# zhangzhousuper/Radish_PT

Measured on AMD Instinct MI355X. Metric: Mrays/s, higher is better.
Workload: dtype f32

## Files before the change

### radish_pt_amd/csrc/device/kernels_wave.h

```cpp
#pragma once
#include "kernels_pt.h"
#include "wg_trace.h"
#include "ray_cull.h"

namespace rd {

constexpr int kWfLitCap = 8192;
constexpr int kWfLitShadow = 0x40000000;
constexpr int kMaxWaveDepth = 32;

struct alignas(128) WaveCounter {
    int v;
    int pad[31];
};
#ifndef RD_WF_TICKET_SHARDS
#define RD_WF_TICKET_SHARDS 8
#endif
constexpr int kTicketShards = RD_WF_TICKET_SHARDS;
struct WaveCounters {
    WaveCounter rayCount[kMaxWaveDepth + 2];
    WaveCounter shadowCount[kMaxWaveDepth + 2];
    WaveCounter litCount[kMaxWaveDepth + 2];
    WaveCounter litShadowCount[kMaxWaveDepth + 2];
    WaveCounter traceHead[kMaxWaveDepth + 2];
    WaveCounter shadeHead[kMaxWaveDepth + 2][4];
    WaveCounter traceTicket[kMaxWaveDepth + 2][kTicketShards];
    WaveCounter shadeTicket[kMaxWaveDepth + 2][kTicketShards];
};

struct WaveWorkspace {
    float4 *ro[2];
    float4 *rd[2];
    float4 *thr[2];
    float4 *prevPos[2];
    float4 *accD;
    float4 *accI;
    float4 *nee[2];
    float4 *sht[2];
    uint2 *rng[2];
    int4 *hit;
    int *rayq[2];
    int *shadowq;
    int *litq[2];
    int litCap;
    int *treeOvf;
    int treeOvfDepth;
#ifdef RD_WF_STAMPS
    unsigned long long *stamps;
    int stampWaves;
    int stampStages;
#endif
    WaveCounters *ctr;
};

constexpr unsigned kWfNeeNone = 2u;
RD_DEV float wfNeeTag(int home, unsigned kind) { return __uint_as_float(((unsigned)home << 2) | kind); }
RD_DEV void wfAddNee(const WaveWorkspace &w, float4 n) {
    const unsigned tag = __float_as_uint(n.w), kind = tag & 3u;
    if (kind == kWfNeeNone) return;
    float4 *acc = (kind == 0u ? w.accD : w.accI) + (tag >> 2);
    const float4 a = *acc;
    *acc = make_float4(a.x + n.x, a.y + n.y, a.z + n.z, 0.f);
}

RD_DEV Ray wfSlotRay(const WaveWorkspace &w, int set, int p, bool shadow, float &limit) {
    if (shadow) {
        const float4 x = w.prevPos[set][p], y = w.sht[set][p];
        return shadowRay(mk3(x.x, x.y, x.z), mk3(y.x, y.y, y.z), limit);
    }
    const float4 o = w.ro[set][p], d = w.rd[set][p];
    limit = 3.402823466e+38f;
    return Ray{mk3(o.x, o.y, o.z), mk3(d.x, d.y, d.z)};
}

struct WaveSlotPath {
    const WaveWorkspace &w;
    const int rs, p;
    const int wr, q;
    int home;
    const bool delta;
    bool nullNee = false;
    RD_DEV v3 throughput() {
        const float4 t = w.thr[rs][p];
        home = __float_as_int(t.w);
        return mk3(t.x, t.y, t.z);
    }
    RD_DEV float samplePdf() const { return w.ro[rs][p].w; }
    RD_DEV bool sampleDelta() const { return delta; }
    RD_DEV v3 prevPos() const { const float4 c = w.prevPos[rs][p]; return mk3(c.x, c.y, c.z); }
    RD_DEV void setDirect(v3 v) { w.accD[home] = make_float4(v.x, v.y, v.z, 0.f); }
    RD_DEV void addIndirect(v3 v) { const float4 a = w.accI[home]; w.accI[home] = make_float4(a.x + v.x, a.y + v.y, a.z + v.z, 0.f); }
    RD_DEV Sampler rng(const DScene &s) const { const uint2 r = w.rng[rs][p]; return Sampler{s.sobol, r.x, (int)r.y}; }
    RD_DEV void setNee(v3 c, float nw) {
        w.nee[wr][q] = make_float4(c.x, c.y, c.z, wfNeeTag(home, nw < 0.f ? kWfNeeNone : (nw == 0.f ? 0u : 1u)));
        nullNee = nw < 0.f || (c.x == 0.f && c.y == 0.f && c.z == 0.f);
    }
    RD_DEV void setPrevPos(v3 x) { w.prevPos[wr][q] = make_float4(x.x, x.y, x.z, 0.f); }
    RD_DEV void setRay(const Ray &ray, float pdf, bool deltaSample, v3 throughput, const Sampler &rng) {
        w.ro[wr][q] = make_float4(ray.o.x, ray.o.y, ray.o.z, pdf);
        w.rd[wr][q] = make_float4(ray.d.x, ray.d.y, ray.d.z, deltaSample ? 1.f : 0.f);
        w.thr[wr][q] = make_float4(throughput.x, throughput.y, throughput.z, __int_as_float(home));
        w.rng[wr][q] = make_uint2(rng.scramble, (unsigned)rng.ptr);
    }
};


RD_DEV void waveAppend(bool pred, int item, int *queue, int *count) {
    unsigned long long mask = __ballot(pred);
    if (mask == 0ull) return;
    int leader = __ffsll((long long)mask) - 1;
    int base = 0;
    if ((int)(threadIdx.x & 63u) == leader) base = atomicAdd(count, __popcll(mask));
    base = __shfl(base, leader, 64);
    if (pred) queue[base + __popcll(mask & laneMaskLt())] = item;
}

constexpr int kShadeChunks = 4;
constexpr int kShadePacket = 64 * kShadeChunks;
RD_DEV void waveAppendN(const bool (&pred)[kShadeChunks], const int (&item)[kShadeChunks], int *queue, int *count) {
    unsigned long long m[kShadeChunks];
    int total = 0;
#pragma unroll
    for (int j = 0; j < kShadeChunks; j++) {
        m[j] = __ballot(pred[j]);
        total += __popcll(m[j]);
    }
    if (total == 0) return;
    int base = 0;
    if ((threadIdx.x & 63u) == 0u) base = atomicAdd(count, total);
    base = __shfl(base, 0, 64);
#pragma unroll
    for (int j = 0; j < kShadeChunks; j++) {
        if (pred[j]) queue[base + __popcll(m[j] & laneMaskLt())] = item[j];
        base += __popcll(m[j]);
    }
}

constexpr int kPacket = 128;
RD_DEV int gridWaves() { return int(gridDim.x * (blockDim.x >> 6)); }
RD_DEV int workgroupTicket(WaveCounter *tickets) {
    __shared__ int ticket;
    if (threadIdx.x == 0) {
        const unsigned x = blockIdx.x % (unsigned)kTicketShards;
        ticket = int(x + (unsigned)kTicketShards * (unsigned)atomicAdd(&tickets[x].v, 1));
    }
    __syncthreads();
    return __builtin_amdgcn_readfirstlane(ticket);
}
RD_DEV int logicalWave(int wg) { return __builtin_amdgcn_readfirstlane(int(wg * int(blockDim.x >> 6) + int(threadIdx.x >> 6))); }
RD_DEV int wavePull(int *head, int packet) {
    int base = 0;
    if ((threadIdx.x & 63u) == 0u) base = atomicAdd(head, packet);
    return __shfl(base, 0, 64) + gridWaves() * packet;
}
RD_DEV int tracePull(int *head, int headBase) {
    int base = 0;
    if ((threadIdx.x & 63u) == 0u) base = atomicAdd(head, kPacket);
    return __builtin_amdgcn_readlane(base, 0) + headBase;
}

RD_DEV unsigned subFrameBlocks(const PixelMap &pm, int part, int parts) { return (unsigned)(pm.numBlocks - part + parts - 1) / (unsigned)parts; }
constexpr int kSobolRows = 10000;
__global__ __launch_bounds__(256) void k_wf_raygen(DScene s, DCamera cam, PixelMap pm, WaveWorkspace w, int looper, int samples, int part,
                                                   int parts) {
    unsigned wg;
    const unsigned nLocal = subFrameBlocks(pm, part, parts);
    const unsigned nGroups = nLocal * (unsigned)samples;
    bool wgValid = xcdSwizzle(blockIdx.x, (nGroups + 3u) >> 2, wg);
    unsigned lane = threadIdx.x & 63u;
    unsigned group = wgValid ? wg * 4u + (threadIdx.x >> 6) : 0xffffffffu / 64u;
    const bool inRange = wgValid && group < nGroups;
    const unsigned b = group / nLocal, blockLocal = group - b * nLocal;
    Pix px = mapPixel(pm, inRange ? blockLocal * (unsigned)parts + (unsigned)part : 0xffffffffu / 64u, lane);
    bool valid = px.valid && inRange;
    int p = int(group * 64u + lane);
    bool listed = false;
    if (valid) {
        Sampler rng = makeSeededRandomEngine(int(((unsigned)looper + b) % (unsigned)kSobolRows), px.index, 0, s.sobol);
        Ray ray = cameraSample(cam, px.x, px.y, sample4D(rng));
        w.ro[0][p] = make_float4(ray.o.x, ray.o.y, ray.o.z, 0.f);
        w.rd[0][p] = make_float4(ray.d.x, ray.d.y, ray.d.z, 0.f);
        w.accD[p] = make_float4(0.f, 0.f, 0.f, 0.f);
        w.accI[p] = make_float4(0.f, 0.f, 0.f, 0.f);
        w.rng[0][p] = make_uint2(rng.scramble, (unsigned)rng.ptr);
        if (fabs_(ray.d.x) < 1.1e-6f || fabs_(ray.d.y) < 1.1e-6f || fabs_(ray.d.z) < 1.1e-6f) {
            const int at = atomicAdd(&w.ctr->litCount[0].v, 1);
            if (at < w.litCap) {
                w.litq[0][at] = p;
                listed = true;
            }
        }
    }
    if (inRange) w.rayq[0][p] = valid ? (listed ? -2 - p : p) : -1;
    if (blockIdx.x == 0 && threadIdx.x == 0) w.ctr->rayCount[0].v = int(nGroups) * 64;
}

#ifndef RD_WF_DUTY_SHARE
#define RD_WF_DUTY_SHARE 0
#endif
#ifndef RD_REFILL_MIN
#define RD_REFILL_MIN 16
#endif
#ifndef RD_WF_FINISH_MIN
#define RD_WF_FINISH_MIN 16
#endif
#ifndef RD_WF_SHADOW_FIRST
#define RD_WF_SHADOW_FIRST 0
#endif
constexpr int kWfStampKinds = 6;
#ifdef RD_WF_STAMPS
#define RD_WF_STAMP(kind) do { if (stampAt && (threadIdx.x & 63u) == 0u) stampAt[kind] = wall_clock64(); } while (0)
#define RD_WF_STAMP_DRY() do { if (exhausted && !stampedDry) { stampedDry = true; RD_WF_STAMP(1); if (stampAt && (threadIdx.x & 63u) == 0u) *headDry = 1ull; } } while (0)
#define RD_WF_STAMP_HELD(held) do { if (stampAt && !stampedHeld && *headDry != 0ull) { \
        stampedHeld = true; const int h_ = (held); if ((threadIdx.x & 63u) == 0u) stampAt[4] = 1ull + (unsigned long long)h_; } } while (0)
#else
#define RD_WF_STAMP(kind) ((void)0)
#define RD_WF_STAMP_DRY() ((void)0)
#define RD_WF_STAMP_HELD(held) ((void)0)
#endif
#ifndef RD_WF_COOP_LONE
#define RD_WF_COOP_LONE 1
#endif

#ifndef RD_WF_TRACE_WAVES
#define RD_WF_TRACE_WAVES 7
#endif
#ifndef RD_WF_PAIR_WAVES
#define RD_WF_PAIR_WAVES 1
#endif
#ifndef RD_WF_PAIR_MAX_WAVES
#define RD_WF_PAIR_MAX_WAVES 6
#endif
template <bool COUNT, bool PAIRS = false>
__global__ __launch_bounds__(256) __attribute__((amdgpu_waves_per_eu(PAIRS && !COUNT ? RD_WF_PAIR_WAVES : (!COUNT ? RD_WF_TRACE_WAVES : 1),
                                                                      PAIRS && !COUNT ? RD_WF_PAIR_MAX_WAVES : 8))) void k_wf_trace(DScene s, WaveWorkspace w, int k) {
    WaveCounters *c = w.ctr;
    const int wg = workgroupTicket(c->traceTicket[k]);
#ifdef RD_WF_STAMPS
    unsigned long long *const stampAt = w.stamps ? w.stamps + ((size_t)k * (size_t)w.stampWaves + (size_t)logicalWave(wg)) * kWfStampKinds : nullptr;
    volatile unsigned long long *const headDry = w.stamps ? w.stamps + (size_t)w.stampStages * (size_t)w.stampWaves * kWfStampKinds + k : nullptr;
    bool stampedDry = false, stampedHeld = false;
    RD_WF_STAMP(0);
#endif
    const int nShadow = (k > 0) ? c->shadowCount[k - 1].v : 0;
    const int nRay = c->rayCount[k].v;
    const int total = nShadow + nRay;
    const int *rayq = w.rayq[k & 1];
    const int set = k & 1;
    WalkStats ws{0, 0};
    unsigned nClosest = 0, nAny = 0, nHits = 0;
    const int end = s.bvhSize;
    const int END = end;

    const int nLit = c->litCount[k].v < w.litCap ? c->litCount[k].v : w.litCap;
    const int dutyGroups = RD_WF_DUTY_SHARE ? 0 : (nLit < int(gridDim.x) ? nLit : int(gridDim.x));
    const bool duty = wg < dutyGroups;
    const int headBase = (int(gridDim.x) - dutyGroups) * int(blockDim.x >> 6) * kPacket;
    int resNext = duty ? headBase : (logicalWave(wg) - dutyGroups * int(blockDim.x >> 6)) * kPacket, resEnd = duty ? resNext : resNext + kPacket;
    bool exhausted = resNext >= total;
    if (resEnd > total) resEnd = total;
    RD_WF_STAMP_DRY();

    bool alive = false;
    bool isShadow = false;
    int p = -1;
    RaySlab rs;
    rs.o = rs.d = rs.inv = mk3(0.f);
    rs.cls = 0;
    const NodeRec *nodes = s.nodes[0];
    int ord = 0, cur = kPairNone;
    PairStack sp{0, 0};
    int node = END, pending = -1;
    float tmax = 0.f;
    int hitPrim = -1;
    v2 hitBary = mk2(0.f, 0.f);
    bool occluded = false;

    constexpr int kStackEntries = PAIRS ? 4 * kPairLds * 64 : 1;
    __shared__ union WfTraceLds {
        WgTraceSharedT<256> wg;
        int2 stack[kStackEntries];
    } lds;
    WgTraceSharedT<256> &wgsh = lds.wg;
    int2 *const stk = lds.stack + (PAIRS ? int(threadIdx.x >> 6) * kPairLds * 64 : 0);
    int2 *const ovf = PAIRS ? reinterpret_cast<int2 *>(w.treeOvf) + (size_t)logicalWave(wg) * (size_t)w.treeOvfDepth * 64 : nullptr;
    for (int it = wg; it < nLit; it += int(gridDim.x)) {
        const int e = w.litq[k & 1][it];
        const bool sh = (e & kWfLitShadow) != 0;
        const int pp = e & (kWfLitShadow - 1);
        float lim;
        const Ray ray = wfSlotRay(w, set, pp, sh, lim);
        const RaySlab urs = makeRaySlab(ray);
        if (urs.cls == 0 || end == 0) continue;
        const NodeRec *un = s.nodes[getMTBVHId(-ray.d)];
        const CoopTrace ct = sh ? wgTraceWhole<true, 256>(s, un, urs, lim, wgsh) : wgTraceWhole<false, 256>(s, un, urs, lim, wgsh);
        if (threadIdx.x == 0) {
            if (sh) {
                nAny++;
                if (!ct.found) wfAddNee(w, w.nee[set][pp]);
            } else {
                nClosest++;
                const bool hit = ct.hitPrim != -1;
                if (hit) nHits++;
                w.hit[pp] = make_int4(ct.hitPrim, __float_as_int(hit ? ct.bary.x : 0.f), __float_as_int(hit ? ct.bary.y : 0.f),
                                      hit ? int(s.primClass[ct.hitPrim]) : 0);
            }
            if (COUNT) {
                ws.nodes += ct.nodes;
                ws.tris += ct.tris;
            }
        }
    }
    RD_WF_STAMP(3);
#ifdef RD_WF_STAMPS
    if (stampAt && (threadIdx.x & 63u) == 0u) stampAt[5] = 1ull + (unsigned long long)nLit;
#endif
    if (PAIRS) __syncthreads();
    bool firstRound = true;
    bool fromList = false;
    for (;;) {
        bool doStart = false;
        fromList = false;
        if (firstRound) {
            firstRound = false;
            const int it = wg + (int(threadIdx.x & 63u) * 4 + int(threadIdx.x >> 6)) * int(gridDim.x);
            if (it < nLit) {
                const int e = w.litq[k & 1][it];
                doStart = true;
                fromList = true;
                isShadow = (e & kWfLitShadow) != 0;
                p = e & (kWfLitShadow - 1);
            }
        }
        unsigned long long idle = __ballot(!alive && !doStart && p < 0);
        int nIdle = __popcll(idle);
        if (!exhausted && nIdle >= RD_REFILL_MIN) {
            RD_WF_STAMP_HELD(resEnd - resNext);
            int myRank = __popcll(idle & laneMaskLt());
            int taken = 0;
            while (taken < nIdle && !exhausted) {
                if (resNext == resEnd) {
                    resNext = tracePull(&c->traceHead[k].v, headBase);
                    resEnd = resNext + kPacket;
                    if (resNext >= total) {
                        exhausted = true;
                        break;
                    }
                    if (resEnd > total) resEnd = total;
                }
                int avail = resEnd - resNext;
                int give = (nIdle - taken) < avail ? (nIdle - taken) : avail;
                if (!alive && !doStart && p < 0 && myRank >= taken && myRank < taken + give) {
                    const int item = resNext + (myRank - taken);
                    doStart = true;
#if RD_WF_SHADOW_FIRST
                    isShadow = item < nShadow;
                    p = isShadow ? w.shadowq[item] : rayq[item - nShadow];
#else
                    isShadow = item >= nRay;
                    p = isShadow ? w.shadowq[item - nRay] : rayq[item];
#endif
                }
                resNext += give;
                taken += give;
            }
        }
        RD_WF_STAMP_DRY();
        if (doStart) {
            if (p >= 0) {
                const Ray ray = wfSlotRay(w, set, p, isShadow, tmax);
                if (isShadow) nAny++;
                else nClosest++;
                rs = makeRaySlab(ray);
                pending = -1;
                if (PAIRS) {
                    ord = getMTBVHId(-ray.d);
                    sp = PairStack{0, 0};
                    if (rs.cls == 0 || end == 0) pairStart<COUNT>(s, rs, tmax, cur, pending, ws);
                    else cur = kPairFresh;
                    alive = true;
                } else {
                    nodes = s.nodes[getMTBVHId(-ray.d)];
                    node = 0;
                    alive = node != END;
                }
                hitPrim = -1;
                occluded = false;
                if (fromList && rs.cls != 0 && end != 0) {
                    if (isShadow) nAny--;
                    else nClosest--;
                    alive = false;
                    p = -1;
                }
            }
        }
        unsigned long long am = __ballot(alive);
        if (am == 0ull) {
            if (exhausted) break;
            continue;
        }

        {
            unsigned long long lit = __ballot(PAIRS ? (alive && cur == kPairFresh) : (alive && rs.cls != 0 && node == 0 && pending < 0));
            while (lit) {
                const int L = __ffsll((long long)lit) - 1;
                lit &= lit - 1ull;
                const bool shadowL = readlaneI(isShadow ? 1 : 0, L) != 0;
                const NodeRec *un = PAIRS ? s.nodes[0] + (size_t)readlaneI(ord, L) * (size_t)(end + 1) : readlanePtr(nodes, L);
                const RaySlab ur = readlaneRay(rs, L);
                const float lim = readlaneF(tmax, L);
                CoopTrace ct = shadowL ? coopTraceWhole<true>(s, un, ur, lim) : coopTraceWhole<false>(s, un, ur, lim);
                if (int(threadIdx.x & 63u) == L) {
                    hitPrim = ct.hitPrim;
                    hitBary = ct.bary;
                    tmax = ct.tmax;
                    occluded = ct.found;
                    node = END;
                    cur = kPairNone;
                    alive = false;
                    if (COUNT) {
                        ws.nodes += ct.nodes;
                        ws.tris += ct.tris;
                    }
                }
            }
        }
        if (PAIRS) {
            bool busy = alive && pending < 0;
            const int nStart = __popcll(__ballot(busy));
            if (nStart > 0) {
                const int minWalk = (nStart * (RD_LEAF_DEN - RD_LEAF_NUM) + RD_LEAF_DEN - 1) / RD_LEAF_DEN;
                const int lane = int(threadIdx.x & 63u);
                do {
                    pairPopOne<COUNT>(stk, lane, ovf, tmax, busy, cur, sp, pending, ws);
                    if (busy && cur >= 0) {
                        pairStep<COUNT>(s.pairs, stk, lane, ovf, rs, tmax, ord, cur, sp, pending, ws);
                        busy = pending < 0 && (cur >= 0 || sp.sp > 0);
                    }
                } while (__popcll(__ballot(busy)) >= (minWalk > 1 ? minWalk : 1));
                alive = alive && (pending >= 0 || cur >= 0 || sp.sp > 0);
            }
        } else
        {
            bool walking = alive && pending < 0;
            const int nStart = __popcll(__ballot(walking));
#if RD_WF_COOP_LONE
            if (nStart == 1) {
                const int L = __ffsll((long long)__ballot(walking)) - 1;
                CoopResult cr = coopWalk(readlanePtr(nodes, L), readlaneI(node, L), end, readlaneRay(rs, L), readlaneF(tmax, L), RD_COOP_WINDOWS);
                if (int(threadIdx.x & 63u) == L) {
                    node = cr.node;
                    pending = cr.pending;
                    if (COUNT) ws.nodes += cr.visited;
                    alive = (node != end) || pending >= 0;
                }
            } else
#endif
            if (nStart > 0) {
                const int minWalk = (nStart * (RD_LEAF_DEN - RD_LEAF_NUM) + RD_LEAF_DEN - 1) / RD_LEAF_DEN;
                do {
                    if (walking) {
                        if (COUNT) ws.nodes++;
                        float4 lo = nodes[node].lo_prim;
                        float4 hi = nodes[node].hi_next;
                        float boundDist;
                        bool boundHit = aabbFast(lo, hi, rs, boundDist);
                        if (boundHit && boundDist < tmax) {
                            pending = __float_as_int(lo.w);
                            node++;
                        } else {
                            node = __float_as_int(hi.w);
                        }
                        walking = pending < 0 && node != END;
                        alive = (node != END) || pending >= 0;
                    }
                } while (__popcll(__ballot(walking)) >= (minWalk > 1 ? minWalk : 1));
            }
        }
        if (alive && pending >= 0) {
            TriVerts t = loadTri(s.tris, pending);
            float dist;
            v2 bary;
            if (COUNT) ws.tris++;
            bool hit = intersectTriangle(rs, t.a, t.b, t.c, bary, dist);
            if (hit && dist < tmax) {
                if (isShadow) {
                    occluded = true;
                    node = END;
                    cur = kPairNone;
                    sp = PairStack{0, 0};
                } else {
                    hitPrim = pending;
                    tmax = dist;
                    hitBary = bary;
                }
            }
            pending = -1;
            alive = PAIRS ? (cur >= 0 || sp.sp > 0) : (node != END);
        }
        const unsigned long long doneM = __ballot(!alive && p >= 0);
        if (doneM != 0ull && __popcll(doneM) * 64 >= (__popcll(doneM) + __popcll(__ballot(alive))) * RD_WF_FINISH_MIN)
        if (!alive && p >= 0) {
            if (isShadow) {
                if (!occluded) wfAddNee(w, w.nee[set][p]);
            } else {
                bool hit = hitPrim != -1;
                if (hit) nHits++;
                w.hit[p] = make_int4(hitPrim, __float_as_int(hit ? hitBary.x : 0.f), __float_as_int(hit ? hitBary.y : 0.f),
                                     hit ? int(s.primClass[hitPrim]) : 0);
            }
            p = -1;
        }
    }
    RD_WF_STAMP(2);
    if (COUNT) flushCounters(s.counters, nClosest, nAny, nHits, ws);
}

constexpr int kSortChunks = 16;
constexpr int kSortPacket = 64 * kSortChunks;
#ifndef RD_WF_SHADE_WAVES
#define RD_WF_SHADE_WAVES 1
#endif
#ifndef RD_WF_CULL_LAST
#define RD_WF_CULL_LAST 1
#endif
#ifndef RD_WF_SKIP_NULL_NEE
#define RD_WF_SKIP_NULL_NEE 1
#endif
__global__ __launch_bounds__(256, RD_WF_SHADE_WAVES) void k_wf_shade(DScene s, WaveWorkspace w, int k, int maxDepth, int sorted,
                                                                     const float4 *__restrict__ emitBox, int walkAll) {
    __shared__ int sSorted[4][kSortPacket];
    WaveCounters *c = w.ctr;
    const bool cullLast = RD_WF_CULL_LAST && !walkAll && k + 1 == maxDepth && !hasEnvMap(s);
    const bool skipNull = RD_WF_SKIP_NULL_NEE && !walkAll;
    float4 boxLo = make_float4(0.f, 0.f, 0.f, 0.f), boxHi = boxLo;
    if (cullLast) {
        boxLo = emitBox[0];
        boxHi = emitBox[1];
    }
    const int wg = workgroupTicket(c->shadeTicket[k]);
    const int lane = int(threadIdx.x & 63u);
    int *mySorted = sSorted[threadIdx.x >> 6];
    {
        const int q = 0;
        const int n = c->rayCount[k].v;
        const int *hitq = w.rayq[k & 1];
        int pendP[kShadeChunks], pendQ[kShadeChunks];
        bool pendShadow[kShadeChunks], pendRay[kShadeChunks];
#pragma unroll
        for (int j = 0; j < kShadeChunks; j++) {
            pendP[j] = pendQ[j] = -1;
            pendShadow[j] = pendRay[j] = false;
        }
        int packet = kShadePacket;
        if (sorted) {
            const int perWave = n / (2 * gridWaves());
            packet = ((perWave + kShadePacket - 1) / kShadePacket) * kShadePacket;
            packet = packet < kShadePacket ? kShadePacket : (packet > kSortPacket ? kSortPacket : packet);
        }
        int packetEnd = 0;
        for (int base = logicalWave(wg) * packet, sub = 0, fresh = 1;;) {
            if (sub == packet) {
                base = wavePull(&c->shadeHead[k][q].v, packet);
                sub = 0;
                fresh = 1;
            }
            if (base + sub >= n) break;
            if (sorted && fresh) {
                fresh = 0;
                packetEnd = (n - base) < packet ? (n - base) : packet;
                int pp[kSortChunks], cls[kSortChunks];
#pragma unroll
                for (int j = 0; j < kSortChunks; j++) {
                    const int i = base + j * 64 + lane;
                    pp[j] = (j * 64 + lane < packetEnd) ? hitq[i] : -1;
                    if (pp[j] <= -2) pp[j] = -2 - pp[j];
                }
#pragma unroll
                for (int j = 0; j < kSortChunks; j++) {
                    cls[j] = (pp[j] >= 0) ? w.hit[pp[j]].w : 0;
                }
                int at = 0;
#pragma unroll
                for (int qq = 0; qq < 4; qq++) {
#pragma unroll
                    for (int j = 0; j < kSortChunks; j++) {
                        const bool in = (j * 64 + lane < packetEnd) && cls[j] == qq;
                        const unsigned long long m = __ballot(in);
                        if (in) mySorted[at + __popcll(m & laneMaskLt())] = pp[j];
                        at += __popcll(m);
                    }
                }
                __builtin_amdgcn_wave_barrier();
            }
            int item = base + sub + lane;
            const int subNow = sub;
            sub += 64;
            bool active = sorted ? (subNow + lane < packetEnd) : (item < n);
            bool emitShadow = false, emitRay = false, litShadow = false, litRay = false, rayFirst = false;
            int p = -1;
            const int q = base + subNow + lane;
            if (active) {
                p = sorted ? mySorted[subNow + lane] : hitq[item];
                if (p <= -2) p = -2 - p;
                active = p >= 0;
            }
            if (active) {
                const int4 h = w.hit[p];
                const float4 rdw = w.rd[k & 1][p];
                WaveSlotPath st{w, k & 1, p, (k + 1) & 1, q, p, rdw.w != 0.f};
                const PathStepResult r = pathStep(s, k, maxDepth, h.x, mk2(__int_as_float(h.y), __int_as_float(h.z)), mk3(rdw.x, rdw.y, rdw.z), st);
                if (r.shadow && !(skipNull && st.nullNee)) {
                    w.sht[(k + 1) & 1][q] = make_float4(r.shadowTo.x, r.shadowTo.y, r.shadowTo.z, 0.f);
                    emitShadow = true;
                    const v3 dl = r.shadowTo - r.shadowFrom;
                    const float l2 = dot(dl, dl) * 1.21e-12f;
                    litShadow = dl.x * dl.x < l2 || dl.y * dl.y < l2 || dl.z * dl.z < l2;
                }
                if (r.extension && !(cullLast && !mayReachEmitters(boxLo, boxHi, r.ray.o, r.ray.d))) {
                    emitRay = true;
                    litRay = fabs_(r.ray.d.x) < 1.1e-6f || fabs_(r.ray.d.y) < 1.1e-6f || fabs_(r.ray.d.z) < 1.1e-6f;
                }
            }
            if (__ballot(litShadow || litRay) != 0ull) {
                int *lq = w.litq[(k + 1) & 1];
                int *lc = &c->litCount[k + 1].v;
                for (int kind = 0; kind < 2; kind++) {
                    const bool pred = kind == 0 ? litShadow : litRay;
                    const unsigned long long m = __ballot(pred);
                    if (m == 0ull) continue;
                    int at = 0;
                    if (lane == 0) at = atomicAdd(lc, __popcll(m));
                    at = __shfl(at, 0, 64) + __popcll(m & laneMaskLt());
                    if (kind == 0) {
                        const int listed = __popcll(__ballot(pred && at < w.litCap));
                        if (lane == 0 && listed > 0) atomicAdd(&c->litShadowCount[k].v, listed);
                    }
                    if (pred && at < w.litCap) {
                        lq[at] = kind == 0 ? (q | kWfLitShadow) : q;
                        if (kind == 0) emitShadow = false;
                        else rayFirst = true;
                    }
                }
            }
            {
                const int j = ((sub >> 6) - 1) & (kShadeChunks - 1);
#pragma unroll
                for (int jj = 0; jj < kShadeChunks; jj++)
                    if (jj == j) {
                        pendP[jj] = q;
                        pendQ[jj] = rayFirst ? -2 - q : q;
                        pendShadow[jj] = emitShadow;
                        pendRay[jj] = emitRay;
                    }
            }
            if ((sub & (kShadePacket - 1)) == 0 || base + sub >= n) {
                waveAppendN(pendShadow, pendP, w.shadowq, &c->shadowCount[k].v);
                waveAppendN(pendRay, pendQ, w.rayq[(k + 1) & 1], &c->rayCount[k + 1].v);
#pragma unroll
                for (int jj = 0; jj < kShadeChunks; jj++) pendShadow[jj] = pendRay[jj] = false;
            }
        }
    }
}

RD_DEV v3 foldRunningMean(v3 mean, float4 acc, int iter) {
    return (mean * float(iter) + finishSample(mk3(acc.x, acc.y, acc.z))) / float(iter + 1);
}
__global__ __launch_bounds__(256) void k_wf_finish(PixelMap pm, WaveWorkspace w, int iter, int samples, float *__restrict__ directIllum,
                                                   float *__restrict__ indirectIllum, int part, int parts) {
    unsigned wg;
    const unsigned nLocal = subFrameBlocks(pm, part, parts);
    bool wgValid = xcdSwizzle(blockIdx.x, (nLocal + 3u) >> 2, wg);
    unsigned lane = threadIdx.x & 63u;
    unsigned blockLocal = wgValid ? wg * 4u + (threadIdx.x >> 6) : 0xffffffffu / 64u;
    const bool inRange = wgValid && blockLocal < nLocal;
    Pix px = mapPixel(pm, inRange ? blockLocal * (unsigned)parts + (unsigned)part : 0xffffffffu / 64u, lane);
    if (!(px.valid && inRange)) return;
    v3 direct = load3(directIllum, px.out), indirect = load3(indirectIllum, px.out);
    for (int b = 0; b < samples; b++) {
        const int p = int(((unsigned)b * nLocal + blockLocal) * 64u + lane);
        direct = foldRunningMean(direct, w.accD[p], iter + b);
        indirect = foldRunningMean(indirect, w.accI[p], iter + b);
    }
    store3(directIllum, px.out, direct);
    store3(indirectIllum, px.out, indirect);
}

}
```

### radish_pt_amd/csrc/radish_hip.hip

```cpp
#include "radish_hip.h"

#include <hip/hip_runtime.h>
#include <dlfcn.h>

#include <algorithm>
#include <cfloat>
#include <climits>
#include <cmath>
#include <cstdarg>
#include <cstdio>
#include <cstring>
#include <mutex>
#include <string>
#include <type_traits>
#include <utility>
#include <vector>

#include "device/kernels_pt.h"
#include "device/kernels_restir.h"
#include "device/kernels_wave.h"
#include "device/kernels_persist.h"
#include "device/kernels_walk.h"
#include "device/kernels_display.h"
#include "device/kernels_denoise.h"
// ... 387 lines not shown
    return f;
}

MatRec toMatRec(const HostMaterial &m) {
    MatRec r;
    r.a = make_float4(asFloat(m.type), m.color[0], m.color[1], m.color[2]);
    r.b = make_float4(m.metallic, m.roughness, m.ior, 0.f);
    r.maps = make_int4(m.map[0], m.map[1], m.map[2], m.map[3]);
    return r;
}

bool mapIdValid(int id, int k, int numTextures) { return id < numTextures && id >= (k == 0 ? -2 : -1); }

bool buildSharedTree(const rdh_scene_desc *d, int S, std::vector<NodeRec> &tree, std::vector<PairRec> &pairs, int &depth) {
    if (S <= 0) return false;
    std::vector<int> canon((size_t)S, -1);
    tree.assign((size_t)S + 1, NodeRec{});
    tree[S].lo_prim = make_float4(0.f, 0.f, 0.f, asFloat(0));
    tree[S].hi_next = make_float4(0.f, 0.f, 0.f, asFloat(0));
    std::vector<int> w3((size_t)S, 0), bits((size_t)S, 0);
    int nextFree = 1;
    std::vector<unsigned char> seen((size_t)S, 0);
    {
        const int32_t *src = d->bvhNodes[0];
        canon[src[1]] = 0;
        for (int p = 0; p < S; p++) {
            const int prim = src[3 * p], box = src[3 * p + 1], next = src[3 * p + 2];
            const int b = canon[box];
            if (b < 0 || seen[b]) return false;
            seen[b] = 1;
            if (prim >= 0) {
                if (next != p + 1) return false;
                w3[b] = prim;
            } else {
                const int first = p + 1;
                if (first >= S) return false;
                const int second = src[3 * first + 2];
                if (second <= first || second >= S || src[3 * second + 2] != next) return false;
                const int bf = src[3 * first + 1], bs = src[3 * second + 1];
                if (bf == bs || canon[bf] >= 0 || canon[bs] >= 0 || nextFree + 2 > S) return false;
                canon[bf] = nextFree;
                canon[bs] = nextFree + 1;
                w3[b] = ~nextFree;
                nextFree += 2;
            }
        }
        if (nextFree != S) return false;
    }
    for (int k = 1; k < 6; k++) {
        const int32_t *src = d->bvhNodes[k];
        std::fill(seen.begin(), seen.end(), 0);
        for (int p = 0; p < S; p++) {
            const int prim = src[3 * p], box = src[3 * p + 1], next = src[3 * p + 2];
            const int b = canon[box];
            if (b < 0 || seen[b]) return false;
            seen[b] = 1;
            if (p == 0 && b != 0) return false;
            if (prim >= 0) {
                if (next != p + 1 || w3[b] != prim) return false;
            } else {
                if (w3[b] >= 0) return false;
                const int first = p + 1;
                if (first >= S) return false;
                const int second = src[3 * first + 2];
                if (second <= first || second >= S || src[3 * second + 2] != next) return false;
                const int c0 = ~w3[b], cf = canon[src[3 * first + 1]], cs = canon[src[3 * second + 1]];
                if (cf == c0 && cs == c0 + 1) {
                } else if (cf == c0 + 1 && cs == c0) {
                    bits[b] |= 1 << k;
                } else {
                    return false;
                }
            }
        }
    }
    depth = 0;
    std::vector<int> pend((size_t)S);
    for (int k = 0; k < 6; k++) {
        pend[0] = 0;
        for (int b = 0; b < S; b++) {
            if (w3[b] >= 0) continue;
            const int c0 = ~w3[b], nb = (bits[b] >> k) & 1;
            pend[c0 + nb] = pend[b] + 1;
            pend[c0 + (nb ^ 1)] = pend[b];
            if (pend[b] + 1 > depth) depth = pend[b] + 1;
        }
    }
    for (int box = 0; box < S; box++) {
        const int b = canon[box];
        const float *q = d->boundingBoxes + 6 * (size_t)box;
        tree[b].lo_prim = make_float4(q[0], q[1], q[2], asFloat(w3[b]));
        tree[b].hi_next = make_float4(q[3], q[4], q[5], asFloat(bits[b]));
    }
    pairs.assign((size_t)(S - 1) / 2 + 1, PairRec{});
    auto childW = [&](int b) { return w3[b] >= 0 ? w3[b] : ~((~w3[b] - 1) / 2); };
    for (int b = 0; b < S; b++) {
        if (w3[b] >= 0) continue;
        const int c0 = ~w3[b], q = (c0 - 1) / 2;
        const float4 l0 = tree[c0].lo_prim, h0 = tree[c0].hi_next, l1 = tree[c0 + 1].lo_prim, h1 = tree[c0 + 1].hi_next;
        pairs[q].lo0_w0 = make_float4(l0.x, l0.y, l0.z, asFloat(childW(c0)));
        pairs[q].hi0_bits = make_float4(h0.x, h0.y, h0.z, asFloat(bits[b]));
        pairs[q].lo1_w1 = make_float4(l1.x, l1.y, l1.z, asFloat(childW(c0 + 1)));
        pairs[q].hi1_pad = make_float4(h1.x, h1.y, h1.z, asFloat(0));
    }
    return true;
}

struct HostCamera {
    int32_t resx, resy;
    float position[3], rotation[3], view[3], up[3], right[3];
    float fov[2], pixelLength[2];
    float rotationMatInv[9];
    float viewProjection[16];
    float lensRadius, focalDist, tanFovY;
};
static_assert(sizeof(HostCamera) == 196, "Camera layout");

DCamera toDeviceCamera(const void *camera196) {
    HostCamera h;
    memcpy(&h, camera196, sizeof(h));
    DCamera d;
    d.resx = h.resx;
    d.resy = h.resy;
    d.position = {h.position[0], h.position[1], h.position[2]};
    d.view = {h.view[0], h.view[1], h.view[2]};
    d.up = {h.up[0], h.up[1], h.up[2]};
    d.right = {h.right[0], h.right[1], h.right[2]};
    d.rotationMatInv.c0 = {h.rotationMatInv[0], h.rotationMatInv[1], h.rotationMatInv[2]};
    d.rotationMatInv.c1 = {h.rotationMatInv[3], h.rotationMatInv[4], h.rotationMatInv[5]};
    d.rotationMatInv.c2 = {h.rotationMatInv[6], h.rotationMatInv[7], h.rotationMatInv[8]};
    d.lensRadius = h.lensRadius;
    d.focalDist = h.focalDist;
    d.tanFovY = tanf(h.fov[1] * 0.01745329251994329576923690768489f);
    return d;
}

PixelMap makePixelMap(const rdh_ctx *c) {
    PixelMap pm;
    pm.W = c->cam.resx;
    pm.H = c->cam.resy;
    pm.tile = c->tile;
    pm.tilesX = (pm.W + pm.tile - 1) / pm.tile;
    int tilesY = (pm.H + pm.tile - 1) / pm.tile;
    pm.numTiles = pm.tilesX * tilesY;
    pm.rank = c->rank;
    pm.world = c->world;
    pm.tilesPerRank = (pm.numTiles + pm.world - 1) / pm.world;
    pm.packed = (c->world > 1 || c->forcePacked) ? 1 : 0;
    int bpe = pm.tile / 8;
    pm.numBlocks = pm.tilesPerRank * bpe * bpe;
    return pm;
}

constexpr int kPairMinNodes = 0;
bool usePairs(const rdh_ctx *c, uint32_t flags) {
    if (!c->scene.ds.pairs || (flags & RDH_PT_NO_PAIRS)) return false;
    if (flags & RDH_PT_PAIRS) return true;
    if (c->pairMode >= 0) return c->pairMode != 0;
    return c->scene.ds.bvhSize >= kPairMinNodes;
}

bool usePackets(uint32_t flags) {
    static const int env = getenv("RADISH_PACKETS") ? atoi(getenv("RADISH_PACKETS")) : 1;
    return env != 0 && !(flags & RDH_PT_NO_PACKETS);
}

unsigned gridFor(const PixelMap &pm) {
    unsigned work = (unsigned)(pm.numBlocks + 3) / 4;
    return ((work + 7u) / 8u) * 8u;
}

unsigned gridBlocks(const PixelMap &pm) { return (((unsigned)pm.numBlocks + 7u) / 8u) * 8u; }

int settleTree(rdh_ctx *c) {
    if (!c->scene.treePending) return RDH_OK;
    HIP_TRY(c, hipEventSynchronize(c->evTree));
    c->scene.treePending = false;
    if (c->scene.treeRefit) {
        c->scene.treeRefit = false;
        if (!c->scene.ds.pairs) return RDH_OK;
        const int4 lo = c->hTreeHdr.as<int4>()[1], hi = c->hTreeHdr.as<int4>()[2];
        c->scene.ds.rootLo = make_float4(__builtin_bit_cast(float, lo.x), __builtin_bit_cast(float, lo.y), __builtin_bit_cast(float, lo.z), c->scene.ds.rootLo.w);
        c->scene.ds.rootHi = make_float4(__builtin_bit_cast(float, hi.x), __builtin_bit_cast(float, hi.y), __builtin_bit_cast(float, hi.z), c->scene.ds.rootHi.w);
        return RDH_OK;
    }
    const int4 *hdr = c->hTreeHdr.as<int4>(), h0 = hdr[0], lo = hdr[1], hi = hdr[2];
    if (h0.y != 0) {
        c->scene.haveScene = false;
        return fail(c, RDH_ERR_STATE, "device BVH build failed (error bits %d); the scene must be uploaded again", h0.y);
    }
    constexpr int kMaxPairDepth = 2048;
    const PairRec *pairs = c->scene.updPairs ? c->scene.updPairs : c->scene.ds.pairs;
    if (h0.x <= kMaxPairDepth) {
        c->scene.ds.pairs = pairs;
        c->scene.ds.treeDepth = h0.x;
        c->scene.ds.rootLo = make_float4(__builtin_bit_cast(float, lo.x), __builtin_bit_cast(float, lo.y), __builtin_bit_cast(float, lo.z),
                                   __builtin_bit_cast(float, lo.w));
        c->scene.ds.rootHi = make_float4(__builtin_bit_cast(float, hi.x), __builtin_bit_cast(float, hi.y), __builtin_bit_cast(float, hi.z),
                                   __builtin_bit_cast(float, hi.w));
    } else {
        c->scene.ds.pairs = nullptr;
        c->scene.ds.treeDepth = 0;
    }
    return RDH_OK;
}

int settleLights(rdh_ctx *c) {
    if (!c->scene.lightsPending) return RDH_OK;
    HIP_TRY(c, hipEventSynchronize(c->evLights));
    c->scene.lightsPending = false;
    c->scene.ds.sumLightPowerInv = c->hLightSums.as<float>()[1];
    return RDH_OK;
}

int requireReady(rdh_ctx *c) {
    if (!c) return RDH_ERR_ARGS;
    if (c->scene.haveScene) {
        int rc = settleTree(c);
        if (rc) return rc;
        if ((rc = settleLights(c))) return rc;
    }
    if (!c->scene.haveScene) return fail(c, RDH_ERR_NO_SCENE, "no scene uploaded (rdh_scene_upload)");
    if (!c->haveCamera) return fail(c, RDH_ERR_NO_SCENE, "no camera set (rdh_set_camera)");
    return RDH_OK;
}

constexpr size_t kProfilePairs = 8192;

long profBegin(rdh_ctx *c, uint32_t flags) {
    if (!(flags & RDH_PT_PROFILE) || c->profUsed >= kProfilePairs) return -1;
    if (c->profEvents.size() < 2 * (c->profUsed + 1)) {
        hipEvent_t a = nullptr, b = nullptr;
        if (newEvent(c, &a, true) || newEvent(c, &b, true)) return -1;
        c->profEvents.push_back(a);
        c->profEvents.push_back(b);
    }
    long i = (long)c->profUsed++;
    hipEventRecord(c->profEvents[2 * i], c->stream);
    return i;
}
void profEnd(rdh_ctx *c, long i) {
    if (i >= 0) hipEventRecord(c->profEvents[2 * i + 1], c->stream);
}

constexpr unsigned kPersistentGrid = 256u * 8u;

template <typename T>
int wfAlloc(rdh_ctx *c, T **out, size_t count) {
    void *p = nullptr;
    HIP_TRY(c, hipMalloc(&p, std::max<size_t>(count * sizeof(T), 16)));
    c->wfAllocs.push_back(p);
    *out = static_cast<T *>(p);
    return RDH_OK;
}

int wavefrontEnsure(rdh_ctx *c, const PixelMap &pm, int samples) {
    long long slots = (long long)pm.numBlocks * 64 * samples;
    if (c->wfCapacity >= slots) return RDH_OK;
    for (void *p : c->wfAllocs) hipFree(p);
    c->wfAllocs.clear();
    c->wfCapacity = 0;
    const size_t n0 = (size_t)slots, n1 = (size_t)((slots / 64 + 1) / 2) * 64;
    for (int h = 0; h < kWfParts; h++) {
        WaveWorkspace &w = c->wf[h];
        const size_t n = h == 0 ? n0 : n1;
        int rc = RDH_OK;
        for (int set = 0; set < 2 && rc == RDH_OK; set++) {
            if ((rc = wfAlloc(c, &w.ro[set], n)) || (rc = wfAlloc(c, &w.rd[set], n)) || (rc = wfAlloc(c, &w.thr[set], n)) ||
                (rc = wfAlloc(c, &w.prevPos[set], n)) || (rc = wfAlloc(c, &w.nee[set], n)) || (rc = wfAlloc(c, &w.sht[set], n)) ||
                (rc = wfAlloc(c, &w.rng[set], n)))
                return rc;
        }
        if ((rc = wfAlloc(c, &w.accD, n)) || (rc = wfAlloc(c, &w.accI, n)) ||
            (rc = wfAlloc(c, &w.hit, n)) || (rc = wfAlloc(c, &w.rayq[0], n)) || (rc = wfAlloc(c, &w.rayq[1], n)) ||
            (rc = wfAlloc(c, &w.shadowq, n)) || (rc = wfAlloc(c, &w.ctr, 1)) || (rc = wfAlloc(c, &w.litq[0], (size_t)kWfLitCap)) ||
            (rc = wfAlloc(c, &w.litq[1], (size_t)kWfLitCap)))
            return rc;
        w.litCap = 0;
    }
    if (!c->evWfFork) {
        int rc;
        if ((rc = newEvent(c, &c->evWfFork)) || (rc = newEvent(c, &c->evWfJoin))) return rc;
        HIP_TRY(c, hipStreamCreateWithFlags(&c->wfStream, hipStreamNonBlocking));
        if ((rc = newEvent(c, &c->evWfJoin3))) return rc;
    }
    c->wfCapacity = slots;
    return RDH_OK;
}

int wavefrontPathTrace(rdh_ctx *c, const PixelMap &pm, float *d_direct, float *d_indirect, int iter, int looper, int samples,
                       int maxDepth, uint32_t flags) {
    if (maxDepth > kMaxWaveDepth) return fail(c, RDH_ERR_ARGS, "maxDepth %d exceeds %d", maxDepth, kMaxWaveDepth);
    const bool count = (flags & RDH_PT_COUNT) != 0, sort = (flags & RDH_PT_SORT_MATERIAL) != 0;
    const bool walkAll = count || (flags & RDH_PT_WALK_ALL) != 0 || c->scene.lightListPartial;
    const bool tree = usePairs(c, flags);
    unsigned traceRes = 0, shadeRes = 0;
    int rq = RDH_OK;
    withBools([&](auto cnt, auto pr) { rq = residentGrid(c, k_wf_trace<cnt.value, pr.value>, 256, &traceRes); }, count, tree);
    if (rq || (rq = residentGrid(c, k_wf_shade, 256, &shadeRes))) return rq;
    if (tree && !count) {
        int cus = 0;
        if (int rc = cuCount(c, &cus)) return rc;
        traceRes = std::min(traceRes, (unsigned)cus * (unsigned)RD_WF_PAIR_MAX_WAVES);
    }
    const unsigned traceGrid = sharedGrid(c, std::min(traceRes, kPersistentGrid), kUnbounded);
    const unsigned shadeGrid = sharedGrid(c, std::min(shadeRes, kPersistentGrid), kUnbounded);
    static const int partsEnv = getenv("RADISH_WF_PARTS") ? atoi(getenv("RADISH_WF_PARTS")) : kWfPartsDefault;
    int parts = ((flags & RDH_PT_WF_SUBFRAMES) && pm.numBlocks >= 2048) ? (partsEnv >= 1 && partsEnv <= kWfParts ? partsEnv : kWfPartsDefault) : 1;
    const int ovfDepth = c->scene.ds.treeDepth + 1;
    const size_t ovfNeed = (size_t)traceGrid * 4 * 64 * (size_t)ovfDepth * 2;
    if (tree && parts > 1 && (size_t)parts * ovfNeed * sizeof(int) > kWfStripBudget) parts = 1;
    hipStream_t sts[kWfParts] = {c->stream, c->sideStream, c->wfStream};
    if (tree) {
        for (int h = 0; h < parts; h++) {
            if (int rc = grow(c, c->wfTreeOvf[h], ovfNeed, ovfNeed * sizeof(int), Busy::Device)) return rc;
            c->wf[h].treeOvf = c->wfTreeOvf[h].as<int>();
            c->wf[h].treeOvfDepth = ovfDepth;
        }
    }
#ifdef RD_WF_STAMPS
    {
        const size_t stamps = (size_t)(maxDepth + 1) * traceGrid * 4 * kWfStampKinds + (size_t)(maxDepth + 1);
        if (int rc = grow(c, c->wfStamps, stamps, stamps * sizeof(unsigned long long), Busy::Device)) return rc;
        HIP_TRY(c, hipMemsetAsync(c->wfStamps.p, 0, stamps * sizeof(unsigned long long), c->stream));
        for (int h = 0; h < kWfParts; h++) {
            c->wf[h].stamps = h == 0 ? c->wfStamps.as<unsigned long long>() : nullptr;
            c->wf[h].stampWaves = (int)(traceGrid * 4);
            c->wf[h].stampStages = maxDepth + 1;
        }
        c->wfStampStages = maxDepth + 1;
        c->wfStampWaves = (int)(traceGrid * 4);
    }
#endif
    if (!c->scene.emitBox)
        if (int rc = sceneAlloc(c, &c->scene.emitBox, 2 * sizeof(float4))) return rc;
    if (RD_WF_CULL_LAST && !walkAll && maxDepth >= 1 && c->scene.ds.envTex < 0) {
        hipLaunchKernelGGL(k_emitter_bounds, dim3(1), dim3(256), 0, c->stream, c->scene.ds.tris, (const int *)c->scene.dLightPrims,
                           c->scene.numLights, c->scene.ds.bvhSize > 0 ? c->scene.ds.nodes[0] : nullptr, c->scene.emitBox);
        HIP_TRY(c, hipGetLastError());
    }
    c->wfLastStages = maxDepth + 1;
    c->wfLastParts = parts;
    const long pf = parts >= 2 ? profBegin(c, flags) : -1;
    if (parts >= 2) {
        HIP_TRY(c, hipEventRecord(c->evWfFork, c->stream));
        for (int h = 1; h < parts; h++) HIP_TRY(c, hipStreamWaitEvent(sts[h], c->evWfFork, 0));
    }
    int rc = RDH_OK;
    auto keep = [&](hipError_t e, const char *what) {
        if (e != hipSuccess && rc == RDH_OK) rc = fail(c, (int)e, "HIP error (%s:%d): %s: %s", __FILE__, __LINE__, what, hipGetErrorString(e));
    };
    for (int h = 0; h < parts; h++) {
        const unsigned waves = traceGrid * 4u;
        c->wf[h].litCap = (int)(waves * 64u < (unsigned)kWfLitCap ? waves * 64u : (unsigned)kWfLitCap);
        if (flags & RDH_PT_WF_SMALL_LISTS) c->wf[h].litCap = 4;
    }
    for (int h = 0; h < parts; h++) {
        hipStream_t st = sts[h];
        WaveWorkspace &w = c->wf[h];
        const unsigned nLocal = (unsigned)(pm.numBlocks - h + parts - 1) / (unsigned)parts;
        const unsigned gridBlk = (((nLocal * (unsigned)samples + 3u) / 4u + 7u) / 8u) * 8u;
        keep(hipMemsetAsync(w.ctr, 0, sizeof(WaveCounters), st), "hipMemsetAsync(wavefront counters)");
        hipLaunchKernelGGL(k_wf_raygen, dim3(gridBlk), dim3(256), 0, st, c->scene.ds, c->cam, pm, w, looper, samples, h, parts);
    }
    for (int k = 0; k <= maxDepth && rc == RDH_OK; k++) {
        for (int h = 0; h < parts; h++) {
            hipStream_t st = sts[h];
            WaveWorkspace &w = c->wf[h];
            long pe = (h == 0 && parts == 1) ? profBegin(c, flags) : -1;
            withBools([&](auto cnt, auto pr) {
                hipLaunchKernelGGL((k_wf_trace<cnt.value, pr.value>), dim3(traceGrid), dim3(256), 0, st, c->scene.ds, w, k);
            }, count, tree);
            profEnd(c, pe);
            hipLaunchKernelGGL(k_wf_shade, dim3(shadeGrid), dim3(256), 0, st, c->scene.ds, w, k, maxDepth, sort ? 1 : 0,
                               (const float4 *)c->scene.emitBox, walkAll ? 1 : 0);
        }
        keep(hipGetLastError(), "wavefront stage launch");
    }
    for (int h = 0; h < parts && rc == RDH_OK; h++) {
        hipStream_t st = sts[h];
        const unsigned nLocal = (unsigned)(pm.numBlocks - h + parts - 1) / (unsigned)parts;
        const unsigned gridBlk = (((nLocal + 3u) / 4u + 7u) / 8u) * 8u;
        hipLaunchKernelGGL(k_wf_finish, dim3(gridBlk), dim3(256), 0, st, pm, c->wf[h], iter, samples, d_direct, d_indirect, h, parts);
    }
    keep(hipGetLastError(), "k_wf_finish");
    if (parts >= 2) {
        hipError_t e1 = hipEventRecord(c->evWfJoin, c->sideStream);
        hipError_t e2 = hipStreamWaitEvent(c->stream, c->evWfJoin, 0);
        hipError_t e3 = hipEventRecord(c->evWfJoin3, c->wfStream);
        hipError_t e4 = hipStreamWaitEvent(c->stream, c->evWfJoin3, 0);
        if (e1 != hipSuccess || e2 != hipSuccess || e3 != hipSuccess || e4 != hipSuccess) {
            hipStreamSynchronize(c->sideStream);
            hipStreamSynchronize(c->wfStream);
            keep(e1 != hipSuccess ? e1 : (e2 != hipSuccess ? e2 : (e3 != hipSuccess ? e3 : e4)), "wavefront join");
        }
    }
    profEnd(c, pf);
    return rc;
}

int ensureStackOverflow(rdh_ctx *c, unsigned resident) {
    const size_t ints = (size_t)resident * 64 * (size_t)(c->scene.ds.treeDepth + 1) * 2;
    return grow(c, c->treeOvf, ints, ints * sizeof(int), Busy::Device);
}

uint32_t resolveStructure(const rdh_ctx *c, const PixelMap &pm, uint32_t flags) {
    if (!(flags & RDH_PT_AUTO)) return flags;
    flags &= ~(RDH_PT_AUTO | RDH_PT_WAVEFRONT | RDH_PT_SORT_MATERIAL | RDH_PT_WF_SUBFRAMES | RDH_PT_PERSISTENT);
    const bool wavefront = c->scene.ds.bvhSize >= 100000 && pm.numBlocks >= 12000;
    return flags | (wavefront ? (RDH_PT_WAVEFRONT | RDH_PT_SORT_MATERIAL | RDH_PT_WF_SUBFRAMES) : RDH_PT_PERSISTENT);
}

int packetBudget(uint32_t flags) { return (flags & RDH_PT_WF_SMALL_LISTS) ? 4 : kPacketBudget; }

int launchWalk(rdh_ctx *c, const float *d_rays, long long n, int4 *d_hits, int *d_occ, bool count, const int *deferCount = nullptr,
               const int *deferList = nullptr, int slotList = 0, bool pairs = false, bool packets = false, int budget = kPacketBudget) {
    const bool any = d_occ != nullptr, defer = deferCount != nullptr;
    packets = packets && !any && n > 0 && (n + 255) / 256 <= 0x7fffffffll;
    if (pairs && !c->scene.ds.pairs) return fail(c, RDH_ERR_UNSUPPORTED, "RDH_PT_PAIRS: the uploaded node arrays are not six orderings of one binary tree, or that tree is more than 2 048 levels deep");
    unsigned resGrid = 0;
    int rc = RDH_OK;
    withBools([&](auto a) {
        rc = pairs ? residentGrid(c, k_walk_pair<false, a.value>, 64, &resGrid) : residentGrid(c, k_walk_persistent<false, a.value>, 64, &resGrid);
    }, any);
    if (rc) return rc;
    const unsigned grid = sharedGrid(c, resGrid, (unsigned long long)((n + 63) / 64));
    const int ovfDepth = c->scene.ds.treeDepth + 1;
    if (pairs && !packets && (rc = ensureStackOverflow(c, resGrid))) return rc;
    int2 *const ovf = c->treeOvf.as<int2>();
    if (!packets) HIP_TRY(c, hipMemsetAsync(c->dPersist, 0, offsetof(PersistCounters, deferred), c->stream));
    if (defer) {
        if ((rc = forkLiteral(c))) return rc;
        withBools([&](auto cnt, auto a) {
            hipLaunchKernelGGL((k_trace_wg_list<cnt.value, a.value>), dim3(kWalkDeferCap), dim3(kWgTraceThreads), 0, c->litStream, c->scene.ds, d_rays, deferList, deferCount, d_hits, d_occ);
        }, count, any);
    }
    if (packets) {
        const unsigned pgrid = (unsigned)((n + 255) / 256);
        withBools([&](auto cnt, auto def) {
            hipLaunchKernelGGL((k_walk_packet<cnt.value, def.value>), dim3(pgrid), dim3(256), 0, c->stream, c->scene.ds, d_rays, n, d_hits, deferCount, slotList, budget);
        }, count, defer);
    } else {
        withBools([&](auto cnt, auto a, auto def) {
            if (pairs)
                hipLaunchKernelGGL((k_walk_pair<cnt.value, a.value, def.value>), dim3(grid), dim3(64), 0, c->stream, c->scene.ds, d_rays, n, d_hits, d_occ,
                                   c->dPersist, ovf, ovfDepth, deferCount, slotList);
            else
                hipLaunchKernelGGL((k_walk_persistent<cnt.value, a.value, def.value>), dim3(grid), dim3(64), 0, c->stream, c->scene.ds, d_rays, n, d_hits, d_occ,
                                   c->dPersist, deferCount, slotList);
        }, count, any, defer);
    }
    if (defer) joinLiteral(c);
    HIP_TRY(c, hipGetLastError());
    return RDH_OK;
}

RestirSplit splitLayout(Carver &k, size_t slots) {
    RestirSplit sp;
    sp.st = k.take<float4>(slots * 48);
    sp.hits = k.take<int4>(slots * 16);
    sp.rays = k.take<float>(slots * 24);
    sp.segs = k.take<float>(slots * 24);
    sp.rawResv = k.take<float>(slots * 36);
    sp.occ = k.take<int>(slots * 4);
    sp.deferCount = k.take<int>(16 + 2 * sizeof(int) * kRestirDeferCap);
    sp.deferList = sp.deferCount + 4;
    return sp;
}

void timeBegin(rdh_ctx *c) {
    hipEventRecord(c->evStart, c->stream);
}
int timeEnd(rdh_ctx *c, const char *what) {
    hipEventRecord(c->evStop, c->stream);
    c->timed = true;
    hipError_t e = hipGetLastError();
    if (e != hipSuccess) return fail(c, (int)e, "HIP error: %s: %s", what, hipGetErrorString(e));
    return RDH_OK;
}

}

extern "C" {

int rdh_create(rdh_ctx **out, int device) {
    if (!out) return RDH_ERR_ARGS;
    *out = nullptr;
    int n = 0;
    if (hipGetDeviceCount(&n) != hipSuccess || n <= 0 || device < 0 || device >= n) return RDH_ERR_NO_DEVICE;
    if (hipSetDevice(device) != hipSuccess) return RDH_ERR_NO_DEVICE;
    rdh_ctx *c = new rdh_ctx;
    c->device = device;
    if (hipStreamCreateWithFlags(&c->ownStream, hipStreamNonBlocking) != hipSuccess ||
        newEvent(c, &c->evStart, true) || newEvent(c, &c->evStop, true) ||
        hipStreamCreateWithFlags(&c->sideStream, hipStreamNonBlocking) != hipSuccess ||
        newEvent(c, &c->evFork) || newEvent(c, &c->evJoin) || newEvent(c, &c->evFrame) || newEvent(c, &c->evSched[0]) ||
        newEvent(c, &c->evSched[1]) ||
        hipMalloc((void **)&c->dCounters, sizeof(Counters)) != hipSuccess ||
        hipMalloc((void **)&c->dPersist, sizeof(PersistCounters)) != hipSuccess) {
        delete c;
        return RDH_ERR_NO_DEVICE;
    }
    c->stream = c->ownStream;
    c->litStream = c->sideStream;
    {
        const char *e = getenv("RADISH_LIT_PRIORITY");
        int least = 0, greatest = 0;
        if (e && atoi(e) != 0 && hipDeviceGetStreamPriorityRange(&least, &greatest) == hipSuccess && greatest < least) {
            hipStream_t hs = nullptr;
            if (hipStreamCreateWithPriority(&hs, hipStreamNonBlocking, greatest) == hipSuccess) c->litStream = hs;
            else (void)hipGetLastError();
        }
    }
    if (hipMemsetAsync(c->dCounters, 0, sizeof(Counters), c->stream) != hipSuccess ||
        hipMemsetAsync(c->dPersist, 0, sizeof(PersistCounters), c->stream) != hipSuccess ||
        hipStreamSynchronize(c->stream) != hipSuccess) {
        delete c;
        return RDH_ERR_NO_DEVICE;
    }
    if (const char *e = getenv("RADISH_PAIRS")) c->pairMode = atoi(e) != 0 ? 1 : 0;
    *out = c;
    return RDH_OK;
}

int rdh_scene_free(rdh_ctx *c) {
    if (!c) return RDH_ERR_ARGS;
    hipSetDevice(c->device);
    hipStreamSynchronize(c->stream);
    for (void *p : c->scene.sceneAllocs) hipFree(p);
    c->scene = SceneState{};
    return RDH_OK;
}

void rdh_destroy(rdh_ctx *c) {
    if (!c) return;
    hipSetDevice(c->device);
    rdh_scene_free(c);
    rdh_restir_free(c);
    rdh_comm_destroy(c);
    for (hipStream_t s : {c->sideStream, c->litStream, c->wfStream, c->commStream})
        if (s) hipStreamSynchronize(s);
    for (void *p : c->wfAllocs) hipFree(p);
    if (c->dCounters) hipFree(c->dCounters);
    if (c->dPersist) hipFree(c->dPersist);
    for (GrowBuf *b : c->bufs) b->release();
    for (hipEvent_t e : c->events) hipEventDestroy(e);
    if (c->litStream && c->litStream != c->sideStream) hipStreamDestroy(c->litStream);
    for (hipStream_t s : {c->wfStream, c->commStream, c->sideStream, c->ownStream})
        if (s) hipStreamDestroy(s);
    delete c;
}

const char *rdh_last_error(const rdh_ctx *c) { return c ? c->err.c_str() : "null context"; }

int rdh_set_stream(rdh_ctx *c, void *s) {
    if (!c) return RDH_ERR_ARGS;
    hipStream_t ns = static_cast<hipStream_t>(s);
    if (ns != c->stream) {
        HIP_TRY(c, hipSetDevice(c->device));
        HIP_TRY(c, hipStreamSynchronize(c->stream));
        if (c->sideStream) HIP_TRY(c, hipStreamSynchronize(c->sideStream));
        if (c->litStream != c->sideStream) HIP_TRY(c, hipStreamSynchronize(c->litStream));
        if (c->wfStream) HIP_TRY(c, hipStreamSynchronize(c->wfStream));
        if (c->commStream) HIP_TRY(c, hipStreamSynchronize(c->commStream));
        c->gbufPending = c->resvPending = false;
        c->orderValid = false;
        c->stream = ns;
    }
    return RDH_OK;
}

int rdh_synchronize(rdh_ctx *c) {
    if (!c) return RDH_ERR_ARGS;
    HIP_TRY(c, hipStreamSynchronize(c->stream));
    if (c->commStream) {
        HIP_TRY(c, hipStreamSynchronize(c->commStream));
        c->gbufPending = c->resvPending = false;
    }
    return RDH_OK;
}

int rdh_scene_upload(rdh_ctx *c, const rdh_scene_desc *d) {
    if (!c || !d) return RDH_ERR_ARGS;
    if (!d->vertices || !d->normals || !d->texcoords || !d->boundingBoxes || !d->materialIds || !d->materials ||
        !d->sampleSequence || d->numPrims <= 0 || d->bvhSize != 2 * d->numPrims - 1 || d->numMaterials <= 0)
        return fail(c, RDH_ERR_ARGS, "rdh_scene_upload: inconsistent descriptor");
    for (int k = 0; k < 6; k++)
        if (!d->bvhNodes[k]) return fail(c, RDH_ERR_ARGS, "rdh_scene_upload: bvhNodes[%d] is null", k);
    if (d->lightSamplerLength > 0 && (!d->lightSampler || !d->lightPrimIds || !d->lightUnitRadiance))
        return fail(c, RDH_ERR_ARGS, "rdh_scene_upload: light arrays missing");
    const bool hasEnv = d->envMapTexId >= 0;
    if (d->lightSamplerLength != d->numLights + (hasEnv ? 1 : 0))
        return fail(c, RDH_ERR_ARGS, "lightSamplerLength %d != numLights %d (+1 with an env map)", d->lightSamplerLength, d->numLights);
    if (d->numTextures < 0 || (d->numTextures > 0 && !d->textures) || d->envMapTexId >= d->numTextures)
        return fail(c, RDH_ERR_ARGS, "rdh_scene_upload: texture table inconsistent");
    if (hasEnv) {
        const rdh_texture &e = d->textures[d->envMapTexId];
        if (!d->envMapSampler || d->envMapSamplerLength != e.width * e.height)
            return fail(c, RDH_ERR_ARGS, "envMapSamplerLength %d != env map %dx%d", d->envMapSamplerLength, e.width, e.height);
    } else if (d->envMapSamplerLength != 0) {
        return fail(c, RDH_ERR_ARGS, "envMapSampler given without envMapTexId");
    }
    HIP_TRY(c, hipSetDevice(c->device));
    rdh_scene_free(c);

    const HostMaterial *hm = static_cast<const HostMaterial *>(d->materials);
// ... 2552 lines not shown
```

Measured before the change: 3327.

## Pack shade pending-emit state into ballot masks and pin shade occupancy

The shade kernel now keeps its pending shadow/ray emissions as per-chunk wave ballot masks instead of per-lane int/bool arrays. Queue entries are reconstructed from the packet's base index and lane. It also switches wave-uniform broadcasts from shfl to readfirstlane. The shade kernel is pinned with amdgpu_waves_per_eu at 4 and its resident grid is capped at CUs×4, which trades register budget and grid size for lower VGPR pressure and higher occupancy. The slot reconstruction assumes each pending chunk's ray index equals first+64*j+lane, which depends on how q maps to sub.

New measurement: 3357 (median of 6 runs). About the same (+0.9%).

```diff
diff --git a/radish_pt_amd/csrc/device/kernels_wave.h b/radish_pt_amd/csrc/device/kernels_wave.h
--- a/radish_pt_amd/csrc/device/kernels_wave.h
+++ b/radish_pt_amd/csrc/device/kernels_wave.h
@@ -117,21 +117,22 @@
 
 constexpr int kShadeChunks = 4;
 constexpr int kShadePacket = 64 * kShadeChunks;
-RD_DEV void waveAppendN(const bool (&pred)[kShadeChunks], const int (&item)[kShadeChunks], int *queue, int *count) {
-    unsigned long long m[kShadeChunks];
+RD_DEV void waveAppendN(const unsigned long long (&m)[kShadeChunks], const unsigned long long (&marked)[kShadeChunks], int first, int *queue,
+                        int *count) {
     int total = 0;
 #pragma unroll
+    for (int j = 0; j < kShadeChunks; j++) total += __popcll(m[j]);
+    if (total == 0) return;
+    const int lane = int(threadIdx.x & 63u);
+    int base = 0;
+    if (lane == 0) base = atomicAdd(count, total);
+    base = __builtin_amdgcn_readfirstlane(base);
+#pragma unroll
     for (int j = 0; j < kShadeChunks; j++) {
-        m[j] = __ballot(pred[j]);
-        total += __popcll(m[j]);
-    }
-    if (total == 0) return;
-    int base = 0;
-    if ((threadIdx.x & 63u) == 0u) base = atomicAdd(count, total);
-    base = __shfl(base, 0, 64);
-#pragma unroll
-    for (int j = 0; j < kShadeChunks; j++) {
-        if (pred[j]) queue[base + __popcll(m[j] & laneMaskLt())] = item[j];
+        if ((m[j] >> lane) & 1ull) {
+            const int slot = first + 64 * j + lane;
+            queue[base + __popcll(m[j] & laneMaskLt())] = ((marked[j] >> lane) & 1ull) ? -2 - slot : slot;
+        }
         base += __popcll(m[j]);
     }
 }
@@ -151,7 +152,7 @@
 RD_DEV int wavePull(int *head, int packet) {
     int base = 0;
     if ((threadIdx.x & 63u) == 0u) base = atomicAdd(head, packet);
-    return __shfl(base, 0, 64) + gridWaves() * packet;
+    return __builtin_amdgcn_readfirstlane(base) + gridWaves() * packet;
 }
 RD_DEV int tracePull(int *head, int headBase) {
     int base = 0;
@@ -519,7 +520,7 @@
 constexpr int kSortChunks = 16;
 constexpr int kSortPacket = 64 * kSortChunks;
 #ifndef RD_WF_SHADE_WAVES
-#define RD_WF_SHADE_WAVES 1
+#define RD_WF_SHADE_WAVES 4
 #endif
 #ifndef RD_WF_CULL_LAST
 #define RD_WF_CULL_LAST 1
@@ -527,8 +528,8 @@
 #ifndef RD_WF_SKIP_NULL_NEE
 #define RD_WF_SKIP_NULL_NEE 1
 #endif
-__global__ __launch_bounds__(256, RD_WF_SHADE_WAVES) void k_wf_shade(DScene s, WaveWorkspace w, int k, int maxDepth, int sorted,
-                                                                     const float4 *__restrict__ emitBox, int walkAll) {
+__global__ __launch_bounds__(256) __attribute__((amdgpu_waves_per_eu(RD_WF_SHADE_WAVES, RD_WF_SHADE_WAVES))) void k_wf_shade(
+    DScene s, WaveWorkspace w, int k, int maxDepth, int sorted, const float4 *__restrict__ emitBox, int walkAll) {
     __shared__ int sSorted[4][kSortPacket];
     WaveCounters *c = w.ctr;
     const bool cullLast = RD_WF_CULL_LAST && !walkAll && k + 1 == maxDepth && !hasEnvMap(s);
@@ -545,13 +546,9 @@
         const int q = 0;
         const int n = c->rayCount[k].v;
         const int *hitq = w.rayq[k & 1];
-        int pendP[kShadeChunks], pendQ[kShadeChunks];
-        bool pendShadow[kShadeChunks], pendRay[kShadeChunks];
-#pragma unroll
-        for (int j = 0; j < kShadeChunks; j++) {
-            pendP[j] = pendQ[j] = -1;
-            pendShadow[j] = pendRay[j] = false;
-        }
+        unsigned long long pendShadow[kShadeChunks], pendRay[kShadeChunks], pendFirst[kShadeChunks];
+#pragma unroll
+        for (int j = 0; j < kShadeChunks; j++) pendShadow[j] = pendRay[j] = pendFirst[j] = 0ull;
         int packet = kShadePacket;
         if (sorted) {
             const int perWave = n / (2 * gridWaves());
@@ -648,17 +645,18 @@
 #pragma unroll
                 for (int jj = 0; jj < kShadeChunks; jj++)
                     if (jj == j) {
-                        pendP[jj] = q;
-                        pendQ[jj] = rayFirst ? -2 - q : q;
-                        pendShadow[jj] = emitShadow;
-                        pendRay[jj] = emitRay;
+                        pendShadow[jj] = __ballot(emitShadow);
+                        pendRay[jj] = __ballot(emitRay);
+                        pendFirst[jj] = __ballot(rayFirst);
                     }
             }
             if ((sub & (kShadePacket - 1)) == 0 || base + sub >= n) {
-                waveAppendN(pendShadow, pendP, w.shadowq, &c->shadowCount[k].v);
-                waveAppendN(pendRay, pendQ, w.rayq[(k + 1) & 1], &c->rayCount[k + 1].v);
-#pragma unroll
-                for (int jj = 0; jj < kShadeChunks; jj++) pendShadow[jj] = pendRay[jj] = false;
+                const int first = base + ((sub - 64) & ~(kShadePacket - 1));
+                const unsigned long long none[kShadeChunks] = {0ull, 0ull, 0ull, 0ull};
+                waveAppendN(pendShadow, none, first, w.shadowq, &c->shadowCount[k].v);
+                waveAppendN(pendRay, pendFirst, first, w.rayq[(k + 1) & 1], &c->rayCount[k + 1].v);
+#pragma unroll
+                for (int jj = 0; jj < kShadeChunks; jj++) pendShadow[jj] = pendRay[jj] = pendFirst[jj] = 0ull;
             }
         }
     }
diff --git a/radish_pt_amd/csrc/radish_hip.hip b/radish_pt_amd/csrc/radish_hip.hip
--- a/radish_pt_amd/csrc/radish_hip.hip
+++ b/radish_pt_amd/csrc/radish_hip.hip
@@ -713,6 +713,11 @@
         int cus = 0;
         if (int rc = cuCount(c, &cus)) return rc;
         traceRes = std::min(traceRes, (unsigned)cus * (unsigned)RD_WF_PAIR_MAX_WAVES);
+    }
+    {
+        int cus = 0;
+        if (int rc = cuCount(c, &cus)) return rc;
+        shadeRes = std::min(shadeRes, (unsigned)cus * (unsigned)RD_WF_SHADE_WAVES);
     }
     const unsigned traceGrid = sharedGrid(c, std::min(traceRes, kPersistentGrid), kUnbounded);
     const unsigned shadeGrid = sharedGrid(c, std::min(shadeRes, kPersistentGrid), kUnbounded);
```
